# zju3dv/RelightableAvatar

Measured on AMD Instinct MI355X. Metric: rays_per_sec, higher is better.
Workload: dtype f16

## Files before the change

### relightableavatar_amd/csrc/ra_api.cpp

```cpp
#include "ra_api_impl.hpp"
#include <cmath>

int check_ready(ra_ctx* c, const char* who) {
    if (!c) { ra_set_error(std::string(who) + ": null ctx"); return 1; }
    if (!c->have_weights) { ra_set_error(std::string(who) + ": weights not finalized"); return 1; }
    if (!c->have_frame) { ra_set_error(std::string(who) + ": no frame set (ra_set_frame)"); return 1; }
    if (hipSetDevice(c->device) != hipSuccess) { ra_set_error(std::string(who) + ": hipSetDevice failed"); return 1; }
    return 0;
}

static void zero_chunk_counters(ra_ctx* c, hipStream_t s) {
    hipMemsetAsync(icnt(c, 0), 0, CNT_ALL * sizeof(int), s);
    c->fc_next = 0;
    c->fc_wrapped = false;
    c->cnt_zero = true;
}
int* next_fine_counter(ra_ctx* c, hipStream_t s) {
    if (c->fc_next >= CNT_FC_SLOTS) {
        hipMemsetAsync(icnt(c, CNT_FC0), 0, CNT_FC_SLOTS * sizeof(int), s);
        c->fc_next = 0;
        c->fc_wrapped = true;
    }
    return icnt(c, CNT_FC0 + c->fc_next++);
}
// ... 100 lines not shown

static void fine_level(ra_ctx* c, const MlpIO& io, int n, bool comp, hipStream_t s, int hint = -1) {
    const int nv = variant_size(n, hint);
    if (comp) {
        Timer t(c, s, T_K3C);
        launch_mlp_sdf_comp(c->host.geo, c->sarena_c.p, c->barena.as<float>(), c->fr, io, nv, s, c->k3cc_ok, grid_size(n, nv));
    } else {
        Timer t(c, s, k3_waves(nv) == 8 ? T_K3_WIDE : T_K3_NARROW);
        k3_launch(c, io, nv, s, grid_size(n, nv));
    }
}

static int hdq_pass(ra_ctx* c, const RaySet& rs, int n, float th, int smooth, float* sdf, hipStream_t s, int what = Q_OTHER,
                    const unsigned char* key = nullptr, int n_key = 0) {
    if (n <= 0) return 0;
    int err = 0;
    int* fine_idx = c->buf<int>("fine_idx", n, &err);
    float* bpts = c->buf<float>("fine_bpts", (size_t)n * 3, &err);
    if (err) return 1;
    HdqOut out{};
    out.sdf = sdf; out.fine_count = next_fine_counter(c, s); out.fine_idx = fine_idx; out.bpts = bpts;
    const int hint = fine_hint(c, c->fc_next - 1);
    int hint2 = -1;
    if (key && n_key > 0) {
        out.key = key;
        out.fine_idx2 = c->buf<int>("fine_idx_k", n_key, &err);
        out.bpts2 = c->buf<float>("fine_bpts_k", (size_t)n_key * 3, &err);
        if (err) return 1;
        out.fine_count2 = next_fine_counter(c, s);
        hint2 = fine_hint(c, c->fc_next - 1);
// ... 64 lines not shown
    ts.t = c->buf<float>(p + "t", n, err);
    ts.d0 = c->buf<float>(p + "d0", n, err);
    ts.occ = c->buf<float>(p + "occ", n, err);
    ts.ot = c->buf<float>(p + "ot", n, err);
    ts.stuck = c->buf<unsigned char>(p + "stuck", n, err);
    if (!soft) {
        ts.dt = c->buf<float>(p + "dt", n, err);
        ts.st = c->buf<float>(p + "st", n, err);
        ts.cd = c->buf<float>(p + "cd", n, err);
        ts.off = c->buf<float>(p + "off", n, err);
        ts.rlx = c->buf<float>(p + "rlx", n, err);
    }
    return ts;
}

int sdf_points_precise(ra_ctx* c, int mode, const float* pts, int n, float dist_th, float* sdf, hipStream_t s) {
    if (n <= 0) return 0;
    if (mode == 2) {
        RaySet rs{};
        rs.mode = 0; rs.x = pts;
        return hdq_pass(c, rs, n, dist_th, 0, sdf, s, Q_PRECISE);
    }
    int err = 0;
    int* idx = c->buf<int>("fine_idx", n, &err);
    if (err) return 1;
    int* cnt = next_fine_counter(c, s);
    launch_iota(idx, n, cnt, s);
    MlpIO io{};
    io.bpts = pts; io.idx = idx; io.count = cnt; io.sdf = sdf; io.dist_th = 1.f; io.smooth = 0;
    io.resd_limit = mode == 0 ? 0.f : c->cfg.resd_limit; io.counters = dcnt(c);
// ... 74 lines not shown
                    int n, const ra_trace_params* p, float* surf, float* occ, float* st, float* ot, void* stream) {
    if (check_ready(c, "ra_sphere_trace")) return 1;
    RA_CHECK(p && n >= 0 && (n == 0 || (ray_o && ray_d && near_ && far_)), "ra_sphere_trace: bad arguments");
    if (n == 0) return 0;
    hipStream_t s = (hipStream_t)stream;
    int err = 0;
    TraceState ts = alloc_trace(c, "tr_", n, false, &err);
    float* sdf = c->buf<float>("tr_sdf", n, &err);
    if (err) return 1;
    ts.near_ = near_; ts.far_ = far_; ts.tan_i = tan_i; ts.light = nullptr;
    launch_trace_init(ts, n, nullptr, *p, s);
    RaySet rs{};
    rs.mode = 1; rs.o = ray_o; rs.d = ray_d; rs.t = ts.t;
    rs.nn_hint = c->buf<int>("tr_nn", (size_t)n * 3, &err);
    if (err) return 1;
    for (int it = 0; it < p->iters; ++it) {
        rs.hint_valid = it > 0;
        if (hdq_pass(c, rs, n, p->dist_th, 1, sdf, s, p->soft_shadow ? Q_OTHER : Q_SURFACE)) return 1;
        launch_trace_update(ts, sdf, n, nullptr, it, *p, s);
    }
    if (occ) RA_HIP(hipMemcpyAsync(occ, ts.occ, (size_t)n * 4, hipMemcpyDeviceToDevice, s));
    if (st) RA_HIP(hipMemcpyAsync(st, ts.st, (size_t)n * 4, hipMemcpyDeviceToDevice, s));
    if (ot) RA_HIP(hipMemcpyAsync(ot, ts.ot, (size_t)n * 4, hipMemcpyDeviceToDevice, s));
    if (surf) {
        float* depth = c->buf<float>("tr_depth", n, &err);
        float* acc = c->buf<float>("tr_acc", n, &err);
        int* hidx = c->buf<int>("tr_hidx", n, &err);
        if (err) return 1;
        launch_surface_finish(ray_o, ray_d, ts.st, ts.occ, n, surf, depth, acc, hidx, icnt(c, CNT_HIT), s);
    }
    RA_HIP(hipGetLastError());
    return 0;
}

// ... 39 lines not shown
        g.ray_light = c->buf<int>("lv_light", NR, &err);
        g.ray_slot = c->buf<int>("lv_slot", NR, &err);
        g.near_ = c->buf<float>("lv_near", NR, &err);
        g.far_ = c->buf<float>("lv_far", NR, &err);
        sh = alloc_trace(c, "sh_", (int)NR, shadow.soft_shadow != 0, &err);
        ssdf = c->buf<float>("sh_sdf", NR, &err);
    }
    const bool keyed = traced && key_tier(c) && c->key_valid;
    const size_t NK = keyed ? (size_t)P * (size_t)(L < KEY_LIGHTS_MAX ? L : KEY_LIGHTS_MAX) : 0;
    if (err) return 1;
    if (c->gate && c->gate->armed) RA_HIP(hipStreamWaitEvent(s, c->gate->done, 0));
    launch_shadow_gen(g, P, s, c->cnt_zero);
    c->cnt_zero = false;
    if (traced) {
        sh.near_ = g.near_; sh.far_ = g.far_; sh.tan_i = c->light_sharp.as<float>(); sh.light = g.ray_light;
        launch_trace_init(sh, (int)NR, g.ray_count, shadow, s);
        RaySet r2{};
        r2.mode = 2; r2.o = st.surf; r2.t = sh.t; r2.pix = g.ray_pix; r2.light = g.ray_light; r2.ldir = c->light_dir.as<float>();
        r2.n_dev = g.ray_count;
        r2.skip = c->cfg.query_skip ? sh.stuck : nullptr;
        r2.nn_hint = c->buf<int>("lv_nn", NR * 3, &err);
        if (err) return 1;
        for (int it = 0; it < shadow.iters; ++it) {
            r2.hint_valid = it > 0;
            r2.hint_src = it == 0 ? st.pix_nn : nullptr;
            r2.hint_src_index = it == 0 ? g.ray_pix : nullptr;
            if (hdq_pass(c, r2, (int)NR, shadow.dist_th, 1, ssdf, s, Q_OTHER, keyed ? c->key_mask.as<unsigned char>() : nullptr, (int)NK)) return 1;
            launch_trace_update(sh, ssdf, (int)NR, g.ray_count, it, shadow, s);
        }
        launch_shadow_scatter(sh.occ, g.ray_slot, g.ray_count, (int)NR, st.lvis, s);
        launch_accumulate(g.ray_count, &dcnt(c)->n_shadow_rays, s);
    }
    if (c->gate) { RA_HIP(hipEventRecord(c->gate->done, s)); c->gate->armed = true; }
    return 0;
}

int ra_begin_render(ra_ctx* c) {
    RA_CHECK(c, "ra_begin_render: null ctx");
    c->call_no = 0;
    return 0;
}

int ra_set_key_probes(ra_ctx* c, const float* probes, int n, int ph, int pw, int accumulate, void* stream) {
    RA_CHECK(c && n >= 0 && (n == 0 || (probes && ph > 0 && pw > 0)), "ra_set_key_probes: bad arguments");
    if (n == 0) { c->key_external = false; c->key_valid = false; return 0; }
    RA_CHECK(c->have_weights && c->n_lights > 0, "ra_set_key_probes: needs the relight network's light set (ra_finalize_weights)");
// ... 65 lines not shown
    int err = 0;
    const int S = p->n_samples, C = raw_channels(c), L = c->n_lights;
    zero_chunk_counters(c, s);
    HintScope hints(c, s);
    const int* perm = nullptr;
    if (bbox && sort_rays(c, "ra_render_sphere_chunk", &ray_o, &ray_d, &near_, &far_, P, bbox, &perm, s)) return 1;
    TraceState ts = alloc_trace(c, "sf_", P, false, &err);
    float* sdf = c->buf<float>("sf_sdf", P, &err);
    float* surf = c->buf<float>("sf_surf", (size_t)P * 3, &err);
    float* depth = c->buf<float>("sf_depth", P, &err);
    float* acc = c->buf<float>("sf_acc", P, &err);
    int* hit_idx = c->buf<int>("sf_hit", P, &err);
    int* slot_of_ray = c->buf<int>("sf_slot", P, &err);
    if (err) return 1;
    ts.near_ = near_; ts.far_ = far_;
    launch_trace_init(ts, P, nullptr, p->surface, s);
    RaySet rs{};
    rs.mode = 1; rs.o = ray_o; rs.d = ray_d; rs.t = ts.t; rs.skip = c->cfg.query_skip ? ts.stuck : nullptr;
    rs.nn_hint = c->buf<int>("sf_nn", (size_t)P * 3, &err);
    if (err) return 1;
    for (int it = 0; it < p->surface.iters; ++it) {
        rs.hint_valid = it > 0;
        if (hdq_pass(c, rs, P, p->surface.dist_th, 1, sdf, s, Q_SURFACE)) return 1;
        launch_trace_update(ts, sdf, P, nullptr, it, p->surface, s);
    }
    int* hit_count = icnt(c, CNT_HIT);
    launch_surface_finish(ray_o, ray_d, ts.st, ts.occ, P, surf, depth, acc, hit_idx, hit_count, s, slot_of_ray, true);
    launch_accumulate(hit_count, &dcnt(c)->n_hit_pixels, s);
    if (relit && sort_hits(c, "ra_render_sphere_chunk", surf, acc, P, bbox, hit_idx, s)) return 1;
    launch_slot_index(hit_idx, hit_count, P, slot_of_ray, s);
    float* xs = c->buf<float>("mt_x", (size_t)P * S * 3, &err);
    float* vs = c->buf<float>("mt_v", (size_t)P * S * 3, &err);
    float* raw = c->buf<float>("mt_raw", (size_t)P * S * C, &err);
    SurfaceMaps m{};
    m.cpts = c->buf<float>("mp_cpts", (size_t)P * 3, &err);
    m.bpts = c->buf<float>("mp_bpts", (size_t)P * 3, &err);
    m.resd = c->buf<float>("mp_resd", (size_t)P * 3, &err);
    m.norm = c->buf<float>("mp_norm", (size_t)P * 3, &err);
    m.albedo = c->buf<float>("mp_albedo", (size_t)P * 3, &err);
    m.rough = c->buf<float>("mp_rough", P, &err);
    m.rgb = c->buf<float>("mp_rgb", (size_t)P * 3, &err);
    m.valbedo = (out->volume_albedo && c->cfg.relight) ? c->buf<float>("mp_valbedo", (size_t)P * 3, &err) : nullptr;
// ... 192 lines not shown
```

### relightableavatar_amd/csrc/ra_api_ctx.cpp

```cpp
#include "ra_api_impl.hpp"
#include <cstdio>
#include <memory>
#include <mutex>

static thread_local std::string g_err;
void ra_set_error(const std::string& msg) { g_err = msg; }

int DevBuf::ensure(size_t need) {
    if (need <= bytes && p) return 0;
    if (need == 0) need = 16;
    if (p) { hipDeviceSynchronize(); hipFree(p); p = nullptr; bytes = 0; }
    size_t want = need + need / 8 + 256;
    hipError_t e = hipMalloc(&p, want);
    if (e != hipSuccess) { ra_set_error(std::string("hipMalloc(") + std::to_string(want) + "): " + hipGetErrorString(e)); p = nullptr; return 1; }
    bytes = want;
    return 0;
}
void DevBuf::release() { if (p) hipFree(p); p = nullptr; bytes = 0; }

ra_ctx::~ra_ctx() {
    for (auto& e : ev_pool) { hipEventDestroy(e.first); hipEventDestroy(e.second); }
    for (int k = 0; k < PinRing::n; ++k) if (pin.ev[k]) hipEventDestroy(pin.ev[k]);
    for (HintSlot& h : hints) { if (h.ev) hipEventDestroy(h.ev); if (h.host) hipHostFree(h.host); }
    if (pin.base) hipHostFree(pin.base);
// ... 1 lines not shown

extern "C" {

const char* ra_last_error(void) { return g_err.c_str(); }
int ra_abi_version(void) { return RA_ABI_VERSION; }

int ra_ctx_create(ra_ctx** out, int device) {
    RA_CHECK(out, "ra_ctx_create: null out");
    int n = 0;
    RA_HIP(hipGetDeviceCount(&n));
    RA_CHECK(n > 0, "ra_ctx_create: no HIP device visible (the render path has no CPU fallback)");
    RA_CHECK(device >= 0 && device < n, "ra_ctx_create: bad device index");
    RA_HIP(hipSetDevice(device));
    std::unique_ptr<ra_ctx> c(new ra_ctx());
    c->device = device;
    if (c->dcounters.ensure(1024)) return 1;
    RA_HIP(hipMemset(c->dcounters.p, 0, 1024));
    *out = c.release();
    return 0;
}

int ra_gate_create(ra_gate** out, int device) {
    RA_CHECK(out, "ra_gate_create: null out");
    RA_HIP(hipSetDevice(device));
    std::unique_ptr<ra_gate> g(new ra_gate());
    g->device = device;
    if (hipEventCreateWithFlags(&g->done, hipEventDisableTiming) != hipSuccess) { g->done = nullptr; ra_set_error("ra_gate_create: hipEventCreate failed"); return 1; }
    *out = g.release();
    return 0;
}
// ... 246 lines not shown
```

### relightableavatar_amd/csrc/ra_ctx.hpp

```cpp
#pragma once
#include "ra_kernels.hpp"
#include <memory>

struct HostNets {
    GeoNet geo{};
    MatNet mat{};
    ColNet col{};
    bool has_color = false;
    float beta = 0.1f;
    std::vector<uint16_t> sarena;
    std::vector<uint16_t> sarena_trim;
    std::vector<uint16_t> sarena_pairs;
    std::vector<uint16_t> sarena_c;
    std::vector<uint16_t> fwd_arena;
    std::vector<uint16_t> bwd_arena;
    int bwd_geo_frags = 0, bwd_frags = 0;
    std::vector<float> shead_row;
    std::vector<float> barena;
    std::vector<float> cond_r0, b_r0, cond_r4, b_r4, cond_c3, b_c3;
    std::vector<float> light_xyz, light_area, light_sharp;
};

struct DevBuf {
    void* p = nullptr;
// ... 92 lines not shown
    DevBuf key_mask, key_share;
    bool key_valid = false;
    bool key_external = false;
    DevBuf lpips_arena;
    std::vector<float> lpips_host;
    bool lpips_loaded = false;
    std::vector<std::unique_ptr<ra_mesh>> meshes;
    std::vector<std::unique_ptr<ra_topo>> topos;
    std::vector<std::unique_ptr<ra_cloth>> cloths;
    int vol_readbacks = 0;
    McQuery mc_query;
    LccQuery lcc_query;
    FrameState fr{};
    DevBuf fvertA, fpverts4, fbias_r0, fbias_r4, fbias_c3, fbvh_pts, fbvh_pairs, fbvh_order;
    bool use_bvh = true;
    DevBuf adj_start, adj_list, adj_dfaces;
    unsigned long long adj_hash = 0;
    int adj_n_faces = 0, adj_n_verts = 0;
    std::map<std::string, DevBuf> scratch;
    DevBuf dcounters;
    int fc_next = 0;
    bool fc_wrapped = false;
    bool cnt_zero = false;
    uint64_t n_shaded = 0;
    bool timing = false;
    std::vector<std::pair<hipEvent_t, hipEvent_t>> ev_pool;
    std::vector<TimerKind> ev_kind;
    size_t ev_used = 0;

    ~ra_ctx();
// ... 10 lines not shown
```

### relightableavatar_amd/csrc/ra_hdq.hip

```cpp
#include "ra_kernels.hpp"
#include <type_traits>
#include <cstdlib>

namespace {

constexpr int KNN_THREADS = 256;

#ifdef RA_COARSE_TS
__device__ long long ra_coarse_ts[64 * 64 * 16 * 8];
extern "C" int ra_coarse_read_timestamps(long long* out) { return (int)hipMemcpyFromSymbol(out, HIP_SYMBOL(ra_coarse_ts), sizeof(ra_coarse_ts)); }
#define RA_CSTAMP(k) do { if (tsp) { __builtin_amdgcn_sched_barrier(0); if ((threadIdx.x & 63) == 0) tsp[k] = __builtin_readcyclecounter(); __builtin_amdgcn_sched_barrier(0); } } while (0)
#else
#define RA_CSTAMP(k) do { } while (0)
#endif
constexpr int VT = 2048;

__device__ __forceinline__ void inv3d(const float R[9], float M[9]) {
    M[0] = R[4] * R[8] - R[7] * R[5];
    M[3] = -R[3] * R[8] + R[6] * R[5];
    M[6] = R[3] * R[7] - R[6] * R[4];
    M[1] = -R[1] * R[8] + R[7] * R[2];
    M[4] = R[0] * R[8] - R[6] * R[2];
    M[7] = -R[0] * R[7] + R[6] * R[1];
    M[2] = R[1] * R[5] - R[4] * R[2];
// ... 194 lines not shown
    if (__builtin_expect(__ballot(d <= d2) == 0ull, 1)) return;
    bool fresh = true;
    if (dedup) fresh = (id != i0) & (id != i1) & (id != i2);
    const bool c2 = fresh && (d < d2 || (d == d2 && id < i2));
    const bool c1 = fresh && (d < d1 || (d == d1 && id < i1));
    const bool c0 = fresh && (d < d0 || (d == d0 && id < i0));
    const float nd2 = c1 ? d1 : (c2 ? d : d2);
    const int ni2 = c1 ? i1 : (c2 ? id : i2);
    const float nd1 = c0 ? d0 : (c1 ? d : d1);
    const int ni1 = c0 ? i0 : (c1 ? id : i1);
    d0 = c0 ? d : d0;
    i0 = c0 ? id : i0;
    d1 = nd1; i1 = ni1; d2 = nd2; i2 = ni2;
}

__device__ __forceinline__ void ray_point(const RaySet& rs, int i, float x[3]) {
    if (rs.mode == 0) {
        x[0] = rs.x[3 * i]; x[1] = rs.x[3 * i + 1]; x[2] = rs.x[3 * i + 2];
    } else if (rs.mode == 1) {
        const float t = rs.t[i];
        x[0] = rs.o[3 * i] + t * rs.d[3 * i];
        x[1] = rs.o[3 * i + 1] + t * rs.d[3 * i + 1];
        x[2] = rs.o[3 * i + 2] + t * rs.d[3 * i + 2];
    } else {
        const float t = rs.t[i];
        const int p = rs.pix[i], l = rs.light[i];
        x[0] = rs.o[3 * p] + t * rs.ldir[3 * l];
        x[1] = rs.o[3 * p + 1] + t * rs.ldir[3 * l + 1];
        x[2] = rs.o[3 * p + 2] + t * rs.ldir[3 * l + 2];
    }
}

template <bool BVH, int SPLIT, bool HINT = false>
__global__ __launch_bounds__(SPLIT == 1 ? KNN_THREADS : 64 * SPLIT) void hdq_coarse_kernel(FrameState fr, RaySet rs, int n_launch, float th, float inv2r2,
                                                                  HdqOut out, int dbg) {
    static_assert(SPLIT == 1 || (BVH && SPLIT >= 2 && SPLIT <= 16), "SPLIT > 1: the workgroup is SPLIT waves on the same 64 queries");
    constexpr int NT = SPLIT == 1 ? KNN_THREADS : 64 * SPLIT;
    __shared__ __attribute__((aligned(16))) unsigned char smem[BVH ? 16 : VT * 16];
#ifdef RA_COARSE_TS
    long long* tsp = blockIdx.x < 64 ? ra_coarse_ts + ((((dbg >> 8) & 63) * 64 + blockIdx.x) * 16 + (threadIdx.x >> 6)) * 8 : nullptr;
    dbg &= 255;
    if (tsp && (threadIdx.x & 63) == 0) { tsp[1] = tsp[2] = tsp[3] = tsp[4] = tsp[5] = tsp[6] = tsp[7] = 0; }
    RA_CSTAMP(0);
#endif
    const int n = rs.n_dev ? min(*rs.n_dev, n_launch) : n_launch;
    const int base = blockIdx.x * (SPLIT == 1 ? KNN_THREADS : 64);
    if (base >= n) return;
    if (blockIdx.x == 0 && threadIdx.x == 0 && out.counters) atomicAdd(&out.counters->n_coarse, (unsigned long long)n);
    const int i = base + (SPLIT == 1 ? threadIdx.x : (threadIdx.x & 63));
    const bool live_q = i < n && !(rs.skip && rs.skip[i < n ? i : 0]);
    bool live = live_q;
    if (__syncthreads_count(live_q) == 0) return;
    float x[3] = {0.f, 0.f, 0.f};
    if (live) ray_point(rs, i, x);
    const float xt[3] = {x[0] - fr.Th[0], x[1] - fr.Th[1], x[2] - fr.Th[2]};
    float p[3];
#pragma unroll
    for (int c = 0; c < 3; ++c) p[c] = xt[0] * fr.R[c] + xt[1] * fr.R[3 + c] + xt[2] * fr.R[6 + c];

    RA_CSTAMP(1);
    float d0 = 3.0e38f, d1 = 3.0e38f, d2 = 3.0e38f;
    int i0 = 0, i1 = 0, i2 = 0;
    if (dbg & 1) { d0 = 1e-4f; d1 = 2e-4f; d2 = 3e-4f; i0 = 0; i1 = 1; i2 = 2; }
    else if (BVH) {
        const int nl = fr.bvh_leaves, ns = fr.bvh_supers;
        if (!live) { d0 = d1 = d2 = -1.f; }
        const unsigned long long lm = __ballot(live);
        const int first = lm ? __ffsll((long long)lm) - 1 : 0;
        const int lane = threadIdx.x & 63;
// ... 277 lines not shown
                      hipStream_t s) {
    hipLaunchKernelGGL(fold_bias_kernel, dim3(64), dim3(256), 0, s, W, ld, col0, ncond, cond, bias, out);
}

int bvh_leaf_count(int n_verts) {
    if (n_verts > BVH_MAXN) return 0;
    return (n_verts + BVH_LEAF - 1) / BVH_LEAF;
}
int bvh_super_count(int n_leaves) { return (n_leaves + BVH_FAN - 1) / BVH_FAN; }

void launch_bvh_build(const float4* pverts4, int n_verts, int* order, float* leaves, float4* sbox, int n_leaves, int n_supers, hipStream_t s) {
    hipLaunchKernelGGL(bvh_rank_kernel, dim3((n_verts + 63) / 64), dim3(BVH_THREADS), 0, s, pverts4, n_verts, order);
    hipLaunchKernelGGL(bvh_boxes_kernel, dim3(1), dim3(BVH_THREADS), 0, s, pverts4, order, n_verts, leaves, sbox, n_leaves, n_supers);
}

void launch_hdq_coarse(const FrameState& fr, const RaySet& rs, int n, float th, float blend_radius, const HdqOut& out,
                       hipStream_t s, bool geodesic) {
    if (n <= 0) return;
    const float inv2r2 = 1.f / (2.f * blend_radius * blend_radius);
    const dim3 grid((n + KNN_THREADS - 1) / KNN_THREADS);
    int dbg = 0, probe = 0, split_max = 196608;
#ifdef RA_TESTING
    static const int e_dbg = getenv("RA_COARSE_DBG") ? atoi(getenv("RA_COARSE_DBG")) : 0;
    static const int e_probe = getenv("RA_COARSE_PROBE") ? atoi(getenv("RA_COARSE_PROBE")) : 0;
    static const int e_split = getenv("RA_COARSE_SPLIT_MAX") ? atoi(getenv("RA_COARSE_SPLIT_MAX")) : 196608;
    dbg = e_dbg; probe = e_probe; split_max = e_split;
#endif
    if (!geodesic) dbg |= 32;
#ifdef RA_COARSE_TS
    static int launch_no = 0;
    dbg |= (launch_no++ & 63) << 8;
#endif
    const bool hint = (rs.nn_hint != nullptr && rs.hint_valid != 0) || rs.hint_src != nullptr;
    for (int pass = probe ? 0 : 1; pass < 2; ++pass) {
        const int d = pass == 0 ? probe : dbg;
        if (fr.bvh_leaves > 0 && n <= split_max)
        {
            const int groups = (n + 63) / 64;
            if (hint) {
                if (n <= split_max / 8) hipLaunchKernelGGL((hdq_coarse_kernel<true, 16, true>), dim3(groups), dim3(1024), 0, s, fr, rs, n, th, inv2r2, out, d);
                else if (n <= split_max / 2) hipLaunchKernelGGL((hdq_coarse_kernel<true, 8, true>), dim3(groups), dim3(512), 0, s, fr, rs, n, th, inv2r2, out, d);
                else hipLaunchKernelGGL((hdq_coarse_kernel<true, 4, true>), dim3(groups), dim3(256), 0, s, fr, rs, n, th, inv2r2, out, d);
            } else {
                if (n <= split_max / 8) hipLaunchKernelGGL((hdq_coarse_kernel<true, 16>), dim3(groups), dim3(1024), 0, s, fr, rs, n, th, inv2r2, out, d);
                else if (n <= split_max / 2) hipLaunchKernelGGL((hdq_coarse_kernel<true, 8>), dim3(groups), dim3(512), 0, s, fr, rs, n, th, inv2r2, out, d);
                else hipLaunchKernelGGL((hdq_coarse_kernel<true, 4>), dim3(groups), dim3(256), 0, s, fr, rs, n, th, inv2r2, out, d);
            }
        }
        else if (fr.bvh_leaves > 0 && hint) hipLaunchKernelGGL((hdq_coarse_kernel<true, 1, true>), grid, dim3(KNN_THREADS), 0, s, fr, rs, n, th, inv2r2, out, d);
        else if (fr.bvh_leaves > 0) hipLaunchKernelGGL((hdq_coarse_kernel<true, 1>), grid, dim3(KNN_THREADS), 0, s, fr, rs, n, th, inv2r2, out, d);
        else hipLaunchKernelGGL((hdq_coarse_kernel<false, 1>), grid, dim3(KNN_THREADS), 0, s, fr, rs, n, th, inv2r2, out, d);
// ... 4 lines not shown
```

### relightableavatar_amd/csrc/ra_kernels.hpp

```cpp
#pragma once
#include "ra_common.hpp"
#include "ra_lpips_pack.hpp"

struct RaySet {
    int mode;
    const float* x;
    const float* o;
    const float* d;
    const float* t;
    const int* pix;
    const int* light;
    const float* ldir;
    const int* n_dev;
    const unsigned char* skip;
    int* nn_hint;
    int hint_valid;
    const int* hint_src;
    const int* hint_src_index;
};

struct HdqOut {
    float* sdf;
    int* fine_count;
    int* fine_idx;
    float* bpts;
    float* mats;
    const unsigned char* key;
    int* fine_count2;
    int* fine_idx2;
    float* bpts2;
    float* raw_zero;
    int raw_C;
    float* dbg_sdf_batch;
// ... 3 lines not shown
    float* dbg_bpts;
    float* dbg_mats;
    DevCounters* counters;
};

void launch_vert_blend(const float* weights, const float* A, const float* big_A, int n_verts, int n_bones, float* vertA,
                       hipStream_t s);
void launch_pack_verts(const float* pverts, int n_verts, float4* out, hipStream_t s);
void launch_fold_bias(const float* W, int ld, int col0, int ncond, const float* cond, const float* bias, float* out,
                      hipStream_t s);
void launch_bvh_build(const float4* pverts4, int n_verts, int* order, float* leaves, float4* sbox, int n_leaves, int n_supers, hipStream_t s);
int bvh_leaf_count(int n_verts);
int bvh_super_count(int n_leaves);
void launch_hdq_coarse(const FrameState& fr, const RaySet& rs, int n, float th, float blend_radius, const HdqOut& out,
                       hipStream_t s, bool geodesic = true);

struct TraceState {
    float *t, *d0, *dt, *st, *ot, *cd, *occ, *off, *rlx;
    const float *near_, *far_;
    const float* tan_i;
    const int* light;
    unsigned char* stuck;
};
void launch_trace_init(const TraceState& ts, int n, const int* n_dev, const ra_trace_params& p, hipStream_t s);

void launch_trace_update(const TraceState& ts, const float* sdf, int n, const int* n_dev, int iter,
                         const ra_trace_params& p, hipStream_t s);

void launch_surface_finish(const float* ray_o, const float* ray_d, const float* st, const float* occ, int P, float* surf,
                           float* depth, float* acc, int* hit_idx, int* hit_count, hipStream_t s, int* slot_of_ray = nullptr,
                           bool counter_is_zero = false);
void launch_slot_index(const int* hit_idx, const int* hit_count, int P, int* slot_of_ray, hipStream_t s);
struct MapJob { const float* src; float* dst; int C; int premul; int src_full; };
constexpr int RA_MAX_MAP_JOBS = 16;
struct EmitMaps { MapJob job[RA_MAX_MAP_JOBS]; long long end[RA_MAX_MAP_JOBS]; int n_jobs; const int* slot_of_ray; const float* acc; const int* perm; int P; };
void launch_emit_maps(const EmitMaps& m, hipStream_t s);
void launch_surface_samples(const float* surf, const float* ray_d, const int* hit_idx, const int* hit_count, int P, int S,
                            float range, float* x, float* v, int* n_out, hipStream_t s);
struct SurfaceMaps {
    float *cpts, *bpts, *resd, *norm, *albedo, *rough, *rgb;
    float* valbedo;
};
void launch_surface_composite(const float* raw, int C, int S, const int* hit_count, int P, int relight, const ra_config& cfg,
                              const SurfaceMaps& m, hipStream_t s);

constexpr int RA_MAX_BOXES = 32;
// ... 407 lines not shown
```

### relightableavatar_amd/csrc/ra_trace.hip

```cpp
#include "ra_kernels.hpp"
#include "ra_shade_dev.hpp"
#include <hipcub/hipcub.hpp>

namespace {

constexpr int TPB = 256;

__device__ __forceinline__ int live_count(const int* n_dev, int n) { return n_dev ? min(*n_dev, n) : n; }

__device__ __forceinline__ float linspace01(int s, int S) {
    if (S == 1) return 0.f;
    const float step = 1.f / (float)(S - 1);
    return (s < S / 2) ? (float)s * step : 1.f - (float)(S - 1 - s) * step;
}

__global__ void trace_init_kernel(TraceState ts, int n_launch, const int* n_dev, float offset, float relax) {
    const int i = blockIdx.x * TPB + threadIdx.x;
    if (i >= live_count(n_dev, n_launch)) return;
    const float nr = ts.near_[i], fr = ts.far_[i];
    ts.t[i] = nr;
    ts.d0[i] = 1e9f;
    ts.occ[i] = 1.f;
    if (ts.stuck) ts.stuck[i] = 0;
    if (ts.dt) ts.dt[i] = 1e9f;
    if (ts.st) ts.st[i] = fr;
    if (ts.ot) ts.ot[i] = fr;
    if (ts.cd) ts.cd[i] = 1e9f;
    if (ts.off) ts.off[i] = offset;
    if (ts.rlx) ts.rlx[i] = relax;
}

template <bool SOFT>
__global__ void trace_update_kernel(TraceState ts, const float* __restrict__ sdf, int n_launch, const int* n_dev, int iter,
                                    ra_trace_params p) {
    const int i = blockIdx.x * TPB + threadIdx.x;
    if (i >= live_count(n_dev, n_launch)) return;
    const float d1 = sdf[i];
    const float d0 = ts.d0[i];
    float t = ts.t[i];
    const float t_prev = t;
    float occ = ts.occ[i];
    const float nr = ts.near_[i], fr = ts.far_[i];
    float tan_i = p.tan_i;
    if (SOFT) {
        const float ti = ts.tan_i ? (ts.light ? ts.tan_i[ts.light[i]] : ts.tan_i[i]) : p.tan_i;
        tan_i = p.tan_i_multiplier * ti;
    }
    const float tan2 = (1.f / tan_i) * 2.f;
    float off = ts.off ? ts.off[i] : p.offset;
    float rlx = ts.rlx ? ts.rlx[i] : p.relax;
    float ot = ts.ot ? ts.ot[i] : 0.f;
    if (SOFT && p.clay_book && iter >= p.shadow_skip_iter) {
        const float dx0 = d0 + rlx * d0 + off;
        const float dx1 = d1 + rlx * d1 + off;
        const float dy = (dx1 * dx1) / (2.f * dx0);
        const float dx = (sqrtf(dx1 * dx1 - dy * dy) - off) / (1.f + rlx);
        const float den = fmaxf(fmaxf(t - dy, nr), p.eps);
        const float cls = fmaxf(dx, 0.f) / den / tan2;
        const bool msk = (cls < occ) && (dy < t) && (dx1 > 0.f) && (dx0 > 0.f) && (dx > 0.f) && (dy > 0.f) && (dy < dx0);
        if (msk) { ot = t - dy; occ = cls; }
    }
    if (iter >= p.shadow_skip_iter) {
        const float cls = fmaxf(d1, 0.f) / fmaxf(fmaxf(t, nr), p.eps) / tan2;
        if (cls < occ) { ot = t; occ = cls; }
    }
    if (!SOFT) {
        const float d1u = fabsf(d1), d0u = fabsf(d0);
        float st = ts.st[i], cd = ts.cd[i];
        const float dt = ts.dt[i];
        const float s0 = (d0 > 0.f) ? 1.f : ((d0 < 0.f) ? -1.f : 0.f);
        const float s1 = (d1 > 0.f) ? 1.f : ((d1 < 0.f) ? -1.f : 0.f);
        if (s0 != s1) {
            st = t - dt * fminf(fmaxf(d1u / (d0u + d1u + p.eps), 0.f), 1.f);
            off = 0.f;
            rlx = 0.f;
        }
        if (d1u < cd) { cd = d1u; st = t; }
        ts.st[i] = st;
        ts.cd[i] = cd;
        ts.off[i] = off;
        ts.rlx[i] = rlx;
    }
    const float dtn = d1 + rlx * d1 + off;
    t = t + dtn;
    t = fminf(t, fr);
    t = fmaxf(t, nr);
    if (ts.dt) ts.dt[i] = dtn;
    ts.t[i] = t;
    if (ts.stuck) ts.stuck[i] = (t == t_prev || (SOFT && occ == 0.f)) ? 1 : 0;
    ts.d0[i] = d1;
    ts.occ[i] = occ;
    if (ts.ot) ts.ot[i] = ot;
}

__global__ void surface_finish_kernel(const float* __restrict__ ro, const float* __restrict__ rd, const float* __restrict__ st,
                                      const float* __restrict__ occ, int P, float* __restrict__ surf, float* __restrict__ depth,
                                      float* __restrict__ acc, int* __restrict__ hit_idx, int* __restrict__ hit_count, int* __restrict__ slot_of_ray) {
    const int i = blockIdx.x * TPB + threadIdx.x;
    bool hit = false;
    if (i < P) {
        if (slot_of_ray) slot_of_ray[i] = -1;
        const float s = st[i];
        const float sx = ro[3 * i] + s * rd[3 * i], sy = ro[3 * i + 1] + s * rd[3 * i + 1], sz = ro[3 * i + 2] + s * rd[3 * i + 2];
        surf[3 * i] = sx; surf[3 * i + 1] = sy; surf[3 * i + 2] = sz;
        depth[i] = (sx - ro[3 * i]) / rd[3 * i];
        const float a = 1.f - occ[i];
        acc[i] = a;
        hit = a > 0.f;
    }
    const unsigned long long m = __ballot(hit);
    if (m == 0ull) return;
    const int lane = threadIdx.x & 63;
    int base = 0;
    if (lane == 0) base = atomicAdd(hit_count, __popcll(m));
    base = __shfl(base, 0);
    if (hit) hit_idx[base + __popcll(m & ((1ull << lane) - 1ull))] = i;
}

__device__ __forceinline__ unsigned expand10t(unsigned v) {
    v = (v * 0x00010001u) & 0xFF0000FFu;
    v = (v * 0x00000101u) & 0x0F00F00Fu;
// ... 589 lines not shown
    if (n <= 0) return;
    hipLaunchKernelGGL(trace_init_kernel, grid_for(n), dim3(TPB), 0, s, ts, n, n_dev, p.offset, p.relax);
}

void launch_trace_update(const TraceState& ts, const float* sdf, int n, const int* n_dev, int iter, const ra_trace_params& p,
                         hipStream_t s) {
    if (n <= 0) return;
    if (p.soft_shadow) hipLaunchKernelGGL(trace_update_kernel<true>, grid_for(n), dim3(TPB), 0, s, ts, sdf, n, n_dev, iter, p);
    else hipLaunchKernelGGL(trace_update_kernel<false>, grid_for(n), dim3(TPB), 0, s, ts, sdf, n, n_dev, iter, p);
}

void launch_surface_finish(const float* ray_o, const float* ray_d, const float* st, const float* occ, int P, float* surf,
                           float* depth, float* acc, int* hit_idx, int* hit_count, hipStream_t s, int* slot_of_ray, bool counter_is_zero) {
    if (!counter_is_zero) hipMemsetAsync(hit_count, 0, sizeof(int), s);
    if (P <= 0) return;
    hipLaunchKernelGGL(surface_finish_kernel, grid_for(P), dim3(TPB), 0, s, ray_o, ray_d, st, occ, P, surf, depth, acc, hit_idx, hit_count, slot_of_ray);
}

void launch_slot_index(const int* hit_idx, const int* hit_count, int P, int* slot_of_ray, hipStream_t s) {
    if (P <= 0) return;
    hipLaunchKernelGGL(slot_index_kernel, grid_for(P), dim3(TPB), 0, s, hit_idx, hit_count, slot_of_ray);
}

void launch_emit_maps(const EmitMaps& m, hipStream_t s) {
    if (m.n_jobs <= 0 || m.P <= 0) return;
    hipLaunchKernelGGL(emit_maps_kernel, grid_for(m.end[m.n_jobs - 1]), dim3(TPB), 0, s, m);
}

void launch_surface_samples(const float* surf, const float* ray_d, const int* hit_idx, const int* hit_count, int P, int S,
                            float range, float* x, float* v, int* n_out, hipStream_t s) {
    if (P <= 0) { hipMemsetAsync(n_out, 0, sizeof(int), s); return; }
// ... 621 lines not shown
```

Baseline: 8.606 million.

## Fuse sphere-trace step update into hinted coarse distance query kernel

Moves the per-iteration trace_update logic into the prologue of the hinted BVH coarse distance-query kernel, and folds the final step into the surface-finish and shadow-finish kernels. Each ray's new t is computed in registers and used directly, so the separate update launch is gone and the stuck flag and t no longer round-trip through memory. Shadow scatter and the ray-count accumulate are merged into one finish kernel. The cost is more registers and extra template instantiations in the coarse kernel, plus an LDS broadcast of t across waves in the split variants.

New measurement: 8.654 million (median of 6 runs). Within noise of the previous version (+0.6%).

```diff
diff --git a/relightableavatar_amd/csrc/ra_api.cpp b/relightableavatar_amd/csrc/ra_api.cpp
--- a/relightableavatar_amd/csrc/ra_api.cpp
+++ b/relightableavatar_amd/csrc/ra_api.cpp
@@ -138,6 +138,7 @@
 static int hdq_pass(ra_ctx* c, const RaySet& rs, int n, float th, int smooth, float* sdf, hipStream_t s, int what = Q_OTHER,
                     const unsigned char* key = nullptr, int n_key = 0) {
     if (n <= 0) return 0;
+    RA_CHECK(rs.step.mode == 0 || hdq_coarse_takes_step(c->fr, rs), "distance query: a trace step needs a hinted pass on the box structure");
     int err = 0;
     int* fine_idx = c->buf<int>("fine_idx", n, &err);
     float* bpts = c->buf<float>("fine_bpts", (size_t)n * 3, &err);
@@ -232,6 +233,15 @@
     return ts;
 }
 
+static bool fused_step(const ra_ctx* c, const ra_trace_params& p) { return c->fused_step && c->fr.bvh_leaves > 0 && p.iters >= 1; }
+static void set_step(RaySet& rs, const TraceState& ts, const ra_trace_params& p, int it, bool use_skip) {
+    rs.step.mode = p.soft_shadow ? 1 : 2;
+    rs.step.iter = it;
+    rs.step.use_skip = use_skip ? 1 : 0;
+    rs.step.ts = ts;
+    rs.step.p = p;
+}
+
 int sdf_points_precise(ra_ctx* c, int mode, const float* pts, int n, float dist_th, float* sdf, hipStream_t s) {
     if (n <= 0) return 0;
     if (mode == 2) {
@@ -336,10 +346,12 @@
     rs.mode = 1; rs.o = ray_o; rs.d = ray_d; rs.t = ts.t;
     rs.nn_hint = c->buf<int>("tr_nn", (size_t)n * 3, &err);
     if (err) return 1;
+    const bool fused = fused_step(c, *p);
     for (int it = 0; it < p->iters; ++it) {
         rs.hint_valid = it > 0;
+        if (fused && it > 0) set_step(rs, ts, *p, it, false);
         if (hdq_pass(c, rs, n, p->dist_th, 1, sdf, s, p->soft_shadow ? Q_OTHER : Q_SURFACE)) return 1;
-        launch_trace_update(ts, sdf, n, nullptr, it, *p, s);
+        if (!fused || it == p->iters - 1) launch_trace_update(ts, sdf, n, nullptr, it, *p, s);
     }
     if (occ) RA_HIP(hipMemcpyAsync(occ, ts.occ, (size_t)n * 4, hipMemcpyDeviceToDevice, s));
     if (st) RA_HIP(hipMemcpyAsync(st, ts.st, (size_t)n * 4, hipMemcpyDeviceToDevice, s));
@@ -409,7 +421,9 @@
     c->cnt_zero = false;
     if (traced) {
         sh.near_ = g.near_; sh.far_ = g.far_; sh.tan_i = c->light_sharp.as<float>(); sh.light = g.ray_light;
-        launch_trace_init(sh, (int)NR, g.ray_count, shadow, s);
+        const bool fused = fused_step(c, shadow);
+        if (fused) sh.stuck = nullptr;
+        if (!fused || !st.pix_nn) launch_trace_init(sh, (int)NR, g.ray_count, shadow, s);
         RaySet r2{};
         r2.mode = 2; r2.o = st.surf; r2.t = sh.t; r2.pix = g.ray_pix; r2.light = g.ray_light; r2.ldir = c->light_dir.as<float>();
         r2.n_dev = g.ray_count;
@@ -420,11 +434,16 @@
             r2.hint_valid = it > 0;
             r2.hint_src = it == 0 ? st.pix_nn : nullptr;
             r2.hint_src_index = it == 0 ? g.ray_pix : nullptr;
+            if (fused && (it > 0 || st.pix_nn)) set_step(r2, sh, shadow, it, c->cfg.query_skip != 0);
             if (hdq_pass(c, r2, (int)NR, shadow.dist_th, 1, ssdf, s, Q_OTHER, keyed ? c->key_mask.as<unsigned char>() : nullptr, (int)NK)) return 1;
-            launch_trace_update(sh, ssdf, (int)NR, g.ray_count, it, shadow, s);
+            if (!fused) launch_trace_update(sh, ssdf, (int)NR, g.ray_count, it, shadow, s);
         }
-        launch_shadow_scatter(sh.occ, g.ray_slot, g.ray_count, (int)NR, st.lvis, s);
-        launch_accumulate(g.ray_count, &dcnt(c)->n_shadow_rays, s);
+        if (fused) {
+            launch_shadow_finish(sh, ssdf, (int)NR, g.ray_count, shadow.iters - 1, shadow, g.ray_slot, st.lvis, &dcnt(c)->n_shadow_rays, s);
+        } else {
+            launch_shadow_scatter(sh.occ, g.ray_slot, g.ray_count, (int)NR, st.lvis, s);
+            launch_accumulate(g.ray_count, &dcnt(c)->n_shadow_rays, s);
+        }
     }
     if (c->gate) { RA_HIP(hipEventRecord(c->gate->done, s)); c->gate->armed = true; }
     return 0;
@@ -520,6 +539,8 @@
     int* slot_of_ray = c->buf<int>("sf_slot", P, &err);
     if (err) return 1;
     ts.near_ = near_; ts.far_ = far_;
+    const bool fused = fused_step(c, p->surface);
+    if (fused) ts.stuck = nullptr;
     launch_trace_init(ts, P, nullptr, p->surface, s);
     RaySet rs{};
     rs.mode = 1; rs.o = ray_o; rs.d = ray_d; rs.t = ts.t; rs.skip = c->cfg.query_skip ? ts.stuck : nullptr;
@@ -527,11 +548,13 @@
     if (err) return 1;
     for (int it = 0; it < p->surface.iters; ++it) {
         rs.hint_valid = it > 0;
+        if (fused && it > 0) set_step(rs, ts, p->surface, it, c->cfg.query_skip != 0);
         if (hdq_pass(c, rs, P, p->surface.dist_th, 1, sdf, s, Q_SURFACE)) return 1;
-        launch_trace_update(ts, sdf, P, nullptr, it, p->surface, s);
+        if (!fused) launch_trace_update(ts, sdf, P, nullptr, it, p->surface, s);
     }
     int* hit_count = icnt(c, CNT_HIT);
-    launch_surface_finish(ray_o, ray_d, ts.st, ts.occ, P, surf, depth, acc, hit_idx, hit_count, s, slot_of_ray, true);
+    if (fused) launch_surface_finish_step(ray_o, ray_d, ts, sdf, p->surface.iters - 1, p->surface, P, surf, depth, acc, hit_idx, hit_count, s, slot_of_ray, true);
+    else launch_surface_finish(ray_o, ray_d, ts.st, ts.occ, P, surf, depth, acc, hit_idx, hit_count, s, slot_of_ray, true);
     launch_accumulate(hit_count, &dcnt(c)->n_hit_pixels, s);
     if (relit && sort_hits(c, "ra_render_sphere_chunk", surf, acc, P, bbox, hit_idx, s)) return 1;
     launch_slot_index(hit_idx, hit_count, P, slot_of_ray, s);
diff --git a/relightableavatar_amd/csrc/ra_api_ctx.cpp b/relightableavatar_amd/csrc/ra_api_ctx.cpp
--- a/relightableavatar_amd/csrc/ra_api_ctx.cpp
+++ b/relightableavatar_amd/csrc/ra_api_ctx.cpp
@@ -1,5 +1,6 @@
 #include "ra_api_impl.hpp"
 #include <cstdio>
+#include <cstdlib>
 #include <memory>
 #include <mutex>
 
@@ -39,6 +40,8 @@
     RA_HIP(hipSetDevice(device));
     std::unique_ptr<ra_ctx> c(new ra_ctx());
     c->device = device;
+    const char* fused = getenv("RA_FUSED_TRACE_STEP");
+    c->fused_step = !(fused && fused[0] == '0' && fused[1] == '\0');
     if (c->dcounters.ensure(1024)) return 1;
     RA_HIP(hipMemset(c->dcounters.p, 0, 1024));
     *out = c.release();
diff --git a/relightableavatar_amd/csrc/ra_ctx.hpp b/relightableavatar_amd/csrc/ra_ctx.hpp
--- a/relightableavatar_amd/csrc/ra_ctx.hpp
+++ b/relightableavatar_amd/csrc/ra_ctx.hpp
@@ -130,6 +130,7 @@
     FrameState fr{};
     DevBuf fvertA, fpverts4, fbias_r0, fbias_r4, fbias_c3, fbvh_pts, fbvh_pairs, fbvh_order;
     bool use_bvh = true;
+    bool fused_step = true;
     DevBuf adj_start, adj_list, adj_dfaces;
     unsigned long long adj_hash = 0;
     int adj_n_faces = 0, adj_n_verts = 0;
diff --git a/relightableavatar_amd/csrc/ra_hdq.hip b/relightableavatar_amd/csrc/ra_hdq.hip
--- a/relightableavatar_amd/csrc/ra_hdq.hip
+++ b/relightableavatar_amd/csrc/ra_hdq.hip
@@ -1,4 +1,5 @@
 #include "ra_kernels.hpp"
+#include "ra_trace_step.hpp"
 #include <type_traits>
 #include <cstdlib>
 
@@ -232,16 +233,17 @@
     d1 = nd1; i1 = ni1; d2 = nd2; i2 = ni2;
 }
 
-__device__ __forceinline__ void ray_point(const RaySet& rs, int i, float x[3]) {
+template <bool FRESH_T = false>
+__device__ __forceinline__ void ray_point(const RaySet& rs, int i, float x[3], float t_fresh = 0.f) {
     if (rs.mode == 0) {
         x[0] = rs.x[3 * i]; x[1] = rs.x[3 * i + 1]; x[2] = rs.x[3 * i + 2];
     } else if (rs.mode == 1) {
-        const float t = rs.t[i];
+        const float t = FRESH_T ? t_fresh : rs.t[i];
         x[0] = rs.o[3 * i] + t * rs.d[3 * i];
         x[1] = rs.o[3 * i + 1] + t * rs.d[3 * i + 1];
         x[2] = rs.o[3 * i + 2] + t * rs.d[3 * i + 2];
     } else {
-        const float t = rs.t[i];
+        const float t = FRESH_T ? t_fresh : rs.t[i];
         const int p = rs.pix[i], l = rs.light[i];
         x[0] = rs.o[3 * p] + t * rs.ldir[3 * l];
         x[1] = rs.o[3 * p + 1] + t * rs.ldir[3 * l + 1];
@@ -249,10 +251,11 @@
     }
 }
 
-template <bool BVH, int SPLIT, bool HINT = false>
+template <bool BVH, int SPLIT, bool HINT = false, int STEP = 0>
 __global__ __launch_bounds__(SPLIT == 1 ? KNN_THREADS : 64 * SPLIT) void hdq_coarse_kernel(FrameState fr, RaySet rs, int n_launch, float th, float inv2r2,
                                                                   HdqOut out, int dbg) {
     static_assert(SPLIT == 1 || (BVH && SPLIT >= 2 && SPLIT <= 16), "SPLIT > 1: the workgroup is SPLIT waves on the same 64 queries");
+    static_assert(STEP == 0 || (BVH && HINT), "a trace step rides on the hinted passes only");
     constexpr int NT = SPLIT == 1 ? KNN_THREADS : 64 * SPLIT;
     __shared__ __attribute__((aligned(16))) unsigned char smem[BVH ? 16 : VT * 16];
 #ifdef RA_COARSE_TS
@@ -266,11 +269,39 @@
     if (base >= n) return;
     if (blockIdx.x == 0 && threadIdx.x == 0 && out.counters) atomicAdd(&out.counters->n_coarse, (unsigned long long)n);
     const int i = base + (SPLIT == 1 ? threadIdx.x : (threadIdx.x & 63));
-    const bool live_q = i < n && !(rs.skip && rs.skip[i < n ? i : 0]);
+    bool live_q;
+    float t_fresh = 0.f;
+    if constexpr (STEP != 0) {
+        constexpr bool SOFT = STEP == 1;
+        __shared__ float step_t[SPLIT > 1 ? 64 : 1];
+        __shared__ unsigned char step_live[SPLIT > 1 ? 64 : 1];
+        const bool mine = i < n && (SPLIT == 1 || threadIdx.x < 64);
+        live_q = false;
+        if (mine) {
+            const TraceState& ts = rs.step.ts;
+            const float nr = ts.near_[i], far = ts.far_[i];
+            TraceRegs r;
+            if (rs.step.iter == 0) {
+                trace_init_regs(r, nr, far, rs.step.p);
+                trace_store_init(ts, i, r);
+            } else {
+                trace_load<SOFT>(ts, i, rs.step.p, r);
+                trace_step<SOFT>(r, out.sdf[i], nr, far, SOFT ? trace_tan_i(ts, i, rs.step.p) : 0.f, rs.step.iter - 1, rs.step.p);
+                trace_store<SOFT>(ts, i, r);
+            }
+            t_fresh = r.t;
+            live_q = !(rs.step.use_skip && r.stuck);
+            if (SPLIT > 1) { step_t[threadIdx.x] = t_fresh; step_live[threadIdx.x] = live_q ? 1 : 0; }
+        }
+        if (__syncthreads_count(live_q) == 0) return;
+        if (SPLIT > 1 && threadIdx.x >= 64 && i < n) { t_fresh = step_t[threadIdx.x & 63]; live_q = step_live[threadIdx.x & 63] != 0; }
+    } else {
+        live_q = i < n && !(rs.skip && rs.skip[i < n ? i : 0]);
+        if (__syncthreads_count(live_q) == 0) return;
+    }
     bool live = live_q;
-    if (__syncthreads_count(live_q) == 0) return;
     float x[3] = {0.f, 0.f, 0.f};
-    if (live) ray_point(rs, i, x);
+    if (live) ray_point<STEP != 0>(rs, i, x, t_fresh);
     const float xt[3] = {x[0] - fr.Th[0], x[1] - fr.Th[1], x[2] - fr.Th[2]};
     float p[3];
 #pragma unroll
@@ -578,6 +609,9 @@
     hipLaunchKernelGGL(bvh_boxes_kernel, dim3(1), dim3(BVH_THREADS), 0, s, pverts4, order, n_verts, leaves, sbox, n_leaves, n_supers);
 }
 
+bool hdq_coarse_hinted(const RaySet& rs) { return (rs.nn_hint != nullptr && rs.hint_valid != 0) || rs.hint_src != nullptr; }
+bool hdq_coarse_takes_step(const FrameState& fr, const RaySet& rs) { return fr.bvh_leaves > 0 && hdq_coarse_hinted(rs); }
+
 void launch_hdq_coarse(const FrameState& fr, const RaySet& rs, int n, float th, float blend_radius, const HdqOut& out,
                        hipStream_t s, bool geodesic) {
     if (n <= 0) return;
@@ -595,10 +629,23 @@
     static int launch_no = 0;
     dbg |= (launch_no++ & 63) << 8;
 #endif
-    const bool hint = (rs.nn_hint != nullptr && rs.hint_valid != 0) || rs.hint_src != nullptr;
+    const bool hint = hdq_coarse_hinted(rs);
+    auto stepped = [&](auto step_, int d) {
+        constexpr int STEP = decltype(step_)::value;
+        const int groups = (n + 63) / 64;
+        if (n > split_max) hipLaunchKernelGGL((hdq_coarse_kernel<true, 1, true, STEP>), grid, dim3(KNN_THREADS), 0, s, fr, rs, n, th, inv2r2, out, d);
+        else if (n <= split_max / 8) hipLaunchKernelGGL((hdq_coarse_kernel<true, 16, true, STEP>), dim3(groups), dim3(1024), 0, s, fr, rs, n, th, inv2r2, out, d);
+        else if (n <= split_max / 2) hipLaunchKernelGGL((hdq_coarse_kernel<true, 8, true, STEP>), dim3(groups), dim3(512), 0, s, fr, rs, n, th, inv2r2, out, d);
+        else hipLaunchKernelGGL((hdq_coarse_kernel<true, 4, true, STEP>), dim3(groups), dim3(256), 0, s, fr, rs, n, th, inv2r2, out, d);
+    };
     for (int pass = probe ? 0 : 1; pass < 2; ++pass) {
         const int d = pass == 0 ? probe : dbg;
-        if (fr.bvh_leaves > 0 && n <= split_max)
+        if (rs.step.mode != 0) {
+            if (pass == 0) continue;
+            if (rs.step.mode == 1) stepped(std::integral_constant<int, 1>{}, d);
+            else stepped(std::integral_constant<int, 2>{}, d);
+        }
+        else if (fr.bvh_leaves > 0 && n <= split_max)
         {
             const int groups = (n + 63) / 64;
             if (hint) {
diff --git a/relightableavatar_amd/csrc/ra_kernels.hpp b/relightableavatar_amd/csrc/ra_kernels.hpp
--- a/relightableavatar_amd/csrc/ra_kernels.hpp
+++ b/relightableavatar_amd/csrc/ra_kernels.hpp
@@ -1,6 +1,22 @@
 #pragma once
 #include "ra_common.hpp"
 #include "ra_lpips_pack.hpp"
+
+struct TraceState {
+    float *t, *d0, *dt, *st, *ot, *cd, *occ, *off, *rlx;
+    const float *near_, *far_;
+    const float* tan_i;
+    const int* light;
+    unsigned char* stuck;
+};
+
+struct TraceStep {
+    int mode;
+    int iter;
+    int use_skip;
+    TraceState ts;
+    ra_trace_params p;
+};
 
 struct RaySet {
     int mode;
@@ -17,6 +33,7 @@
     int hint_valid;
     const int* hint_src;
     const int* hint_src_index;
+    TraceStep step;
 };
 
 struct HdqOut {
@@ -50,14 +67,9 @@
 int bvh_super_count(int n_leaves);
 void launch_hdq_coarse(const FrameState& fr, const RaySet& rs, int n, float th, float blend_radius, const HdqOut& out,
                        hipStream_t s, bool geodesic = true);
-
-struct TraceState {
-    float *t, *d0, *dt, *st, *ot, *cd, *occ, *off, *rlx;
-    const float *near_, *far_;
-    const float* tan_i;
-    const int* light;
-    unsigned char* stuck;
-};
+bool hdq_coarse_hinted(const RaySet& rs);
+bool hdq_coarse_takes_step(const FrameState& fr, const RaySet& rs);
+
 void launch_trace_init(const TraceState& ts, int n, const int* n_dev, const ra_trace_params& p, hipStream_t s);
 
 void launch_trace_update(const TraceState& ts, const float* sdf, int n, const int* n_dev, int iter,
@@ -66,6 +78,11 @@
 void launch_surface_finish(const float* ray_o, const float* ray_d, const float* st, const float* occ, int P, float* surf,
                            float* depth, float* acc, int* hit_idx, int* hit_count, hipStream_t s, int* slot_of_ray = nullptr,
                            bool counter_is_zero = false);
+void launch_surface_finish_step(const float* ray_o, const float* ray_d, const TraceState& ts, const float* sdf, int iter, const ra_trace_params& p,
+                                int P, float* surf, float* depth, float* acc, int* hit_idx, int* hit_count, hipStream_t s,
+                                int* slot_of_ray = nullptr, bool counter_is_zero = false);
+void launch_shadow_finish(const TraceState& ts, const float* sdf, int n, const int* n_dev, int iter, const ra_trace_params& p, const int* ray_slot,
+                          float* lvis, unsigned long long* n_rays_total, hipStream_t s);
 void launch_slot_index(const int* hit_idx, const int* hit_count, int P, int* slot_of_ray, hipStream_t s);
 struct MapJob { const float* src; float* dst; int C; int premul; int src_full; };
 constexpr int RA_MAX_MAP_JOBS = 16;
diff --git a/relightableavatar_amd/csrc/ra_trace.hip b/relightableavatar_amd/csrc/ra_trace.hip
--- a/relightableavatar_amd/csrc/ra_trace.hip
+++ b/relightableavatar_amd/csrc/ra_trace.hip
@@ -1,5 +1,6 @@
 #include "ra_kernels.hpp"
 #include "ra_shade_dev.hpp"
+#include "ra_trace_step.hpp"
 #include <hipcub/hipcub.hpp>
 
 namespace {
@@ -35,76 +36,50 @@
                                     ra_trace_params p) {
     const int i = blockIdx.x * TPB + threadIdx.x;
     if (i >= live_count(n_dev, n_launch)) return;
-    const float d1 = sdf[i];
-    const float d0 = ts.d0[i];
-    float t = ts.t[i];
-    const float t_prev = t;
-    float occ = ts.occ[i];
-    const float nr = ts.near_[i], fr = ts.far_[i];
-    float tan_i = p.tan_i;
-    if (SOFT) {
-        const float ti = ts.tan_i ? (ts.light ? ts.tan_i[ts.light[i]] : ts.tan_i[i]) : p.tan_i;
-        tan_i = p.tan_i_multiplier * ti;
-    }
-    const float tan2 = (1.f / tan_i) * 2.f;
-    float off = ts.off ? ts.off[i] : p.offset;
-    float rlx = ts.rlx ? ts.rlx[i] : p.relax;
-    float ot = ts.ot ? ts.ot[i] : 0.f;
-    if (SOFT && p.clay_book && iter >= p.shadow_skip_iter) {
-        const float dx0 = d0 + rlx * d0 + off;
-        const float dx1 = d1 + rlx * d1 + off;
-        const float dy = (dx1 * dx1) / (2.f * dx0);
-        const float dx = (sqrtf(dx1 * dx1 - dy * dy) - off) / (1.f + rlx);
-        const float den = fmaxf(fmaxf(t - dy, nr), p.eps);
-        const float cls = fmaxf(dx, 0.f) / den / tan2;
-        const bool msk = (cls < occ) && (dy < t) && (dx1 > 0.f) && (dx0 > 0.f) && (dx > 0.f) && (dy > 0.f) && (dy < dx0);
-        if (msk) { ot = t - dy; occ = cls; }
-    }
-    if (iter >= p.shadow_skip_iter) {
-        const float cls = fmaxf(d1, 0.f) / fmaxf(fmaxf(t, nr), p.eps) / tan2;
-        if (cls < occ) { ot = t; occ = cls; }
-    }
-    if (!SOFT) {
-        const float d1u = fabsf(d1), d0u = fabsf(d0);
-        float st = ts.st[i], cd = ts.cd[i];
-        const float dt = ts.dt[i];
-        const float s0 = (d0 > 0.f) ? 1.f : ((d0 < 0.f) ? -1.f : 0.f);
-        const float s1 = (d1 > 0.f) ? 1.f : ((d1 < 0.f) ? -1.f : 0.f);
-        if (s0 != s1) {
-            st = t - dt * fminf(fmaxf(d1u / (d0u + d1u + p.eps), 0.f), 1.f);
-            off = 0.f;
-            rlx = 0.f;
-        }
-        if (d1u < cd) { cd = d1u; st = t; }
-        ts.st[i] = st;
-        ts.cd[i] = cd;
-        ts.off[i] = off;
-        ts.rlx[i] = rlx;
-    }
-    const float dtn = d1 + rlx * d1 + off;
-    t = t + dtn;
-    t = fminf(t, fr);
-    t = fmaxf(t, nr);
-    if (ts.dt) ts.dt[i] = dtn;
-    ts.t[i] = t;
-    if (ts.stuck) ts.stuck[i] = (t == t_prev || (SOFT && occ == 0.f)) ? 1 : 0;
-    ts.d0[i] = d1;
-    ts.occ[i] = occ;
-    if (ts.ot) ts.ot[i] = ot;
-}
-
+    TraceRegs r;
+    trace_load<SOFT>(ts, i, p, r);
+    trace_step<SOFT>(r, sdf[i], ts.near_[i], ts.far_[i], SOFT ? trace_tan_i(ts, i, p) : 0.f, iter, p);
+    trace_store<SOFT>(ts, i, r);
+}
+
+template <bool SOFT>
+__global__ void shadow_finish_kernel(TraceState ts, const float* __restrict__ sdf, int n_launch, const int* __restrict__ n_dev, int iter,
+                                     ra_trace_params p, const int* __restrict__ ray_slot, float* __restrict__ lvis,
+                                     unsigned long long* __restrict__ n_rays_total) {
+    const int i = blockIdx.x * TPB + threadIdx.x;
+    if (i == 0) atomicAdd(n_rays_total, (unsigned long long)*n_dev);
+    if (i >= live_count(n_dev, n_launch)) return;
+    TraceRegs r;
+    trace_load<SOFT>(ts, i, p, r);
+    trace_step<SOFT>(r, sdf[i], ts.near_[i], ts.far_[i], SOFT ? trace_tan_i(ts, i, p) : 0.f, iter, p);
+    lvis[ray_slot[i]] = r.occ;
+}
+
+template <int STEP>
 __global__ void surface_finish_kernel(const float* __restrict__ ro, const float* __restrict__ rd, const float* __restrict__ st,
                                       const float* __restrict__ occ, int P, float* __restrict__ surf, float* __restrict__ depth,
-                                      float* __restrict__ acc, int* __restrict__ hit_idx, int* __restrict__ hit_count, int* __restrict__ slot_of_ray) {
+                                      float* __restrict__ acc, int* __restrict__ hit_idx, int* __restrict__ hit_count, int* __restrict__ slot_of_ray,
+                                      TraceState ts, const float* __restrict__ sdf, int iter, ra_trace_params p) {
     const int i = blockIdx.x * TPB + threadIdx.x;
     bool hit = false;
     if (i < P) {
         if (slot_of_ray) slot_of_ray[i] = -1;
-        const float s = st[i];
+        float s, oc;
+        if constexpr (STEP != 0) {
+            constexpr bool SOFT = STEP == 1;
+            TraceRegs r;
+            trace_load<SOFT>(ts, i, p, r);
+            trace_step<SOFT>(r, sdf[i], ts.near_[i], ts.far_[i], SOFT ? trace_tan_i(ts, i, p) : 0.f, iter, p);
+            s = SOFT ? ts.st[i] : r.st;
+            oc = r.occ;
+        } else {
+            s = st[i];
+            oc = occ[i];
+        }
         const float sx = ro[3 * i] + s * rd[3 * i], sy = ro[3 * i + 1] + s * rd[3 * i + 1], sz = ro[3 * i + 2] + s * rd[3 * i + 2];
         surf[3 * i] = sx; surf[3 * i + 1] = sy; surf[3 * i + 2] = sz;
         depth[i] = (sx - ro[3 * i]) / rd[3 * i];
-        const float a = 1.f - occ[i];
+        const float a = 1.f - oc;
         acc[i] = a;
         hit = a > 0.f;
     }
@@ -724,7 +699,26 @@
                            float* depth, float* acc, int* hit_idx, int* hit_count, hipStream_t s, int* slot_of_ray, bool counter_is_zero) {
     if (!counter_is_zero) hipMemsetAsync(hit_count, 0, sizeof(int), s);
     if (P <= 0) return;
-    hipLaunchKernelGGL(surface_finish_kernel, grid_for(P), dim3(TPB), 0, s, ray_o, ray_d, st, occ, P, surf, depth, acc, hit_idx, hit_count, slot_of_ray);
+    hipLaunchKernelGGL(surface_finish_kernel<0>, grid_for(P), dim3(TPB), 0, s, ray_o, ray_d, st, occ, P, surf, depth, acc, hit_idx, hit_count, slot_of_ray,
+                       TraceState{}, nullptr, 0, ra_trace_params{});
+}
+
+void launch_surface_finish_step(const float* ray_o, const float* ray_d, const TraceState& ts, const float* sdf, int iter, const ra_trace_params& p,
+                                int P, float* surf, float* depth, float* acc, int* hit_idx, int* hit_count, hipStream_t s, int* slot_of_ray,
+                                bool counter_is_zero) {
+    if (!counter_is_zero) hipMemsetAsync(hit_count, 0, sizeof(int), s);
+    if (P <= 0) return;
+    if (p.soft_shadow) hipLaunchKernelGGL(surface_finish_kernel<1>, grid_for(P), dim3(TPB), 0, s, ray_o, ray_d, nullptr, nullptr, P, surf, depth, acc, hit_idx,
+                                          hit_count, slot_of_ray, ts, sdf, iter, p);
+    else hipLaunchKernelGGL(surface_finish_kernel<2>, grid_for(P), dim3(TPB), 0, s, ray_o, ray_d, nullptr, nullptr, P, surf, depth, acc, hit_idx, hit_count,
+                            slot_of_ray, ts, sdf, iter, p);
+}
+
+void launch_shadow_finish(const TraceState& ts, const float* sdf, int n, const int* n_dev, int iter, const ra_trace_params& p, const int* ray_slot,
+                          float* lvis, unsigned long long* n_rays_total, hipStream_t s) {
+    if (n <= 0) return;
+    if (p.soft_shadow) hipLaunchKernelGGL(shadow_finish_kernel<true>, grid_for(n), dim3(TPB), 0, s, ts, sdf, n, n_dev, iter, p, ray_slot, lvis, n_rays_total);
+    else hipLaunchKernelGGL(shadow_finish_kernel<false>, grid_for(n), dim3(TPB), 0, s, ts, sdf, n, n_dev, iter, p, ray_slot, lvis, n_rays_total);
 }
 
 void launch_slot_index(const int* hit_idx, const int* hit_count, int P, int* slot_of_ray, hipStream_t s) {
diff --git a/relightableavatar_amd/csrc/ra_trace_step.hpp b/relightableavatar_amd/csrc/ra_trace_step.hpp
--- /dev/null
+++ b/relightableavatar_amd/csrc/ra_trace_step.hpp
@@ -0,0 +1,117 @@
+#pragma once
+#include "ra_kernels.hpp"
+
+struct TraceRegs {
+    float t, d0, occ, ot;
+    float dt, st, cd;
+    float off, rlx;
+    bool stuck;
+};
+
+__device__ __forceinline__ void trace_init_regs(TraceRegs& r, float nr, float fr, const ra_trace_params& p) {
+    r.t = nr; r.d0 = 1e9f; r.occ = 1.f; r.ot = fr;
+    r.dt = 1e9f; r.st = fr; r.cd = 1e9f;
+    r.off = p.offset; r.rlx = p.relax;
+    r.stuck = false;
+}
+
+template <bool SOFT>
+__device__ __forceinline__ void trace_load(const TraceState& ts, int i, const ra_trace_params& p, TraceRegs& r) {
+    r.d0 = ts.d0[i];
+    r.t = ts.t[i];
+    r.occ = ts.occ[i];
+    r.off = ts.off ? ts.off[i] : p.offset;
+    r.rlx = ts.rlx ? ts.rlx[i] : p.relax;
+    r.ot = ts.ot ? ts.ot[i] : 0.f;
+    r.dt = 0.f; r.st = 0.f; r.cd = 0.f;
+    if (!SOFT) { r.st = ts.st[i]; r.cd = ts.cd[i]; r.dt = ts.dt[i]; }
+    r.stuck = false;
+}
+
+__device__ __forceinline__ float trace_tan_i(const TraceState& ts, int i, const ra_trace_params& p) {
+    return ts.tan_i ? (ts.light ? ts.tan_i[ts.light[i]] : ts.tan_i[i]) : p.tan_i;
+}
+
+template <bool SOFT>
+__device__ __forceinline__ void trace_step(TraceRegs& r, float d1, float nr, float fr, float ti, int iter, const ra_trace_params& p) {
+    const float d0 = r.d0;
+    float t = r.t;
+    const float t_prev = t;
+    float occ = r.occ;
+    float tan_i = p.tan_i;
+    if (SOFT) tan_i = p.tan_i_multiplier * ti;
+    const float tan2 = (1.f / tan_i) * 2.f;
+    float off = r.off;
+    float rlx = r.rlx;
+    float ot = r.ot;
+    if (SOFT && p.clay_book && iter >= p.shadow_skip_iter) {
+        const float dx0 = d0 + rlx * d0 + off;
+        const float dx1 = d1 + rlx * d1 + off;
+        const float dy = (dx1 * dx1) / (2.f * dx0);
+        const float dx = (sqrtf(dx1 * dx1 - dy * dy) - off) / (1.f + rlx);
+        const float den = fmaxf(fmaxf(t - dy, nr), p.eps);
+        const float cls = fmaxf(dx, 0.f) / den / tan2;
+        const bool msk = (cls < occ) && (dy < t) && (dx1 > 0.f) && (dx0 > 0.f) && (dx > 0.f) && (dy > 0.f) && (dy < dx0);
+        if (msk) { ot = t - dy; occ = cls; }
+    }
+    if (iter >= p.shadow_skip_iter) {
+        const float cls = fmaxf(d1, 0.f) / fmaxf(fmaxf(t, nr), p.eps) / tan2;
+        if (cls < occ) { ot = t; occ = cls; }
+    }
+    if (!SOFT) {
+        const float d1u = fabsf(d1), d0u = fabsf(d0);
+        float st = r.st, cd = r.cd;
+        const float dt = r.dt;
+        const float s0 = (d0 > 0.f) ? 1.f : ((d0 < 0.f) ? -1.f : 0.f);
+        const float s1 = (d1 > 0.f) ? 1.f : ((d1 < 0.f) ? -1.f : 0.f);
+        if (s0 != s1) {
+            st = t - dt * fminf(fmaxf(d1u / (d0u + d1u + p.eps), 0.f), 1.f);
+            off = 0.f;
+            rlx = 0.f;
+        }
+        if (d1u < cd) { cd = d1u; st = t; }
+        r.st = st;
+        r.cd = cd;
+        r.off = off;
+        r.rlx = rlx;
+    }
+    const float dtn = d1 + rlx * d1 + off;
+    t = t + dtn;
+    t = fminf(t, fr);
+    t = fmaxf(t, nr);
+    r.dt = dtn;
+    r.t = t;
+    r.stuck = (t == t_prev || (SOFT && occ == 0.f));
+    r.d0 = d1;
+    r.occ = occ;
+    r.ot = ot;
+}
+
+__device__ __forceinline__ void trace_store_init(const TraceState& ts, int i, const TraceRegs& r) {
+    ts.t[i] = r.t;
+    ts.d0[i] = r.d0;
+    ts.occ[i] = r.occ;
+    if (ts.stuck) ts.stuck[i] = 0;
+    if (ts.dt) ts.dt[i] = r.dt;
+    if (ts.st) ts.st[i] = r.st;
+    if (ts.ot) ts.ot[i] = r.ot;
+    if (ts.cd) ts.cd[i] = r.cd;
+    if (ts.off) ts.off[i] = r.off;
+    if (ts.rlx) ts.rlx[i] = r.rlx;
+}
+
+template <bool SOFT>
+__device__ __forceinline__ void trace_store(const TraceState& ts, int i, const TraceRegs& r) {
+    if (!SOFT) {
+        ts.st[i] = r.st;
+        ts.cd[i] = r.cd;
+        ts.off[i] = r.off;
+        ts.rlx[i] = r.rlx;
+    }
+    if (ts.dt) ts.dt[i] = r.dt;
+    ts.t[i] = r.t;
+    if (ts.stuck) ts.stuck[i] = r.stuck ? 1 : 0;
+    ts.d0[i] = r.d0;
+    ts.occ[i] = r.occ;
+    if (ts.ot) ts.ot[i] = r.ot;
+}
```
